# at-aaims/OmniFed

Measured on AMD Instinct MI355X. Metric: GB/s device-resident QSGD encode+decode, Llama-400M grads, 1/2/4/8 GPUs, higher is better.
Workload: dtype f32; 1 GPU; llama400m QSGD encode+decode, bit_width 4 (16 levels, int8 wire), philox draws, client weighting fused (alpha = batch_samples = rank + 1), one client per GPU; tensors=183, elements_per_client=401122304, bit_width=4, parallelism=clients1

## Files before the change

### omnifed_amd/csrc/omf_common.h

```cpp
#pragma once

#include <hip/hip_runtime.h>
#include <stdint.h>

#include <cstdlib>
#include <string>

namespace omf {

constexpr int kThreads = 256;
constexpr int kWaves = kThreads / 64;

constexpr unsigned kOrderEventFlags = hipEventDisableTiming | hipEventDisableSystemFence;

struct TopkStats {
  int64_t calls = 0, exact = 0;
};

struct TopkKnobs {
  TopkStats stats;
  bool init = false;
  int32_t groups = 1;
  int32_t dbg = 0;
  int32_t force_fallback = 0;
  int64_t sample_runs = 0;
  float sure_z = 1.5f, sure_c = 2.0f;
  bool scatter_small = true;
  bool planned_scatter = true;
};

inline const char* knob(const char* name) {
#ifdef OMF_EXPERIMENTS
  return std::getenv(name);
#else
  (void)name;
  return nullptr;
#endif
}

void set_error(const std::string& msg);
int fail(int code, const std::string& msg);
int hip_fail(hipError_t e, const char* what);

#define OMF_HIP(call)                                   \
  do {                                                  \
    hipError_t e_ = (call);                             \
    if (e_ != hipSuccess) return ::omf::hip_fail(e_, #call); \
  } while (0)

struct DeviceGuard {
  int prev = -1;
  bool ok = false;
  explicit DeviceGuard(int dev) {
    if (hipGetDevice(&prev) != hipSuccess) prev = -1;
    ok = hipSetDevice(dev) == hipSuccess;
  }
  ~DeviceGuard() {
    if (prev >= 0) (void)hipSetDevice(prev);
  }
};


__device__ __forceinline__ double wave_sum_f64(double v) {
#pragma unroll
  for (int o = 32; o > 0; o >>= 1) v += __shfl_xor(v, o, 64);
  return v;
}

__device__ __forceinline__ double block_sum_f64(double v, double* lds ) {
  v = wave_sum_f64(v);
  const int lane = threadIdx.x & 63, wave = threadIdx.x >> 6;
  if (lane == 0) lds[wave] = v;
  __syncthreads();
  double s = lds[0];
#pragma unroll
  for (int w = 1; w < kWaves; ++w) s += lds[w];
  __syncthreads();
  return s;
}

__device__ __forceinline__ uint64_t ld_agent(const uint64_t* p) {
  return __hip_atomic_load(const_cast<uint64_t*>(p), __ATOMIC_RELAXED, __HIP_MEMORY_SCOPE_AGENT);
}
__device__ __forceinline__ void st_agent(uint64_t* p, uint64_t v) {
  __hip_atomic_store(p, v, __ATOMIC_RELAXED, __HIP_MEMORY_SCOPE_AGENT);
}
__device__ __forceinline__ uint32_t add_agent(uint32_t* p, uint32_t v) {
  return __hip_atomic_fetch_add(p, v, __ATOMIC_RELAXED, __HIP_MEMORY_SCOPE_AGENT);
}
__device__ __forceinline__ void drain_vmem() { asm volatile("s_waitcnt vmcnt(0)" ::: "memory"); }

#ifndef OMF_PHILOX_ROUNDS
#define OMF_PHILOX_ROUNDS 10
#endif
__device__ __forceinline__ uint4 philox4x32_10(uint4 c, uint32_t k0, uint32_t k1) {
#pragma unroll
  for (int r = 0; r < OMF_PHILOX_ROUNDS; ++r) {
    if (r) {
      k0 += 0x9E3779B9u;
      k1 += 0xBB67AE85u;
    }
    const uint64_t p0 = (uint64_t)0xD2511F53u * c.x;
    const uint64_t p1 = (uint64_t)0xCD9E8D57u * c.z;
    c = make_uint4(__builtin_amdgcn_bitop3_b32((uint32_t)(p1 >> 32), c.y, k0, 0x96), (uint32_t)p1,
                   __builtin_amdgcn_bitop3_b32((uint32_t)(p0 >> 32), c.w, k1, 0x96), (uint32_t)p0);
  }
  return c;
}

__device__ __forceinline__ float u24(uint32_t w) { return (float)(w & 0xFFFFFFu) * 5.9604644775390625e-08f; }

__device__ __forceinline__ float4 u24x4(uint32_t w0, uint32_t w1, uint32_t w2) {
  return make_float4(u24(w0), u24(__builtin_amdgcn_alignbit(w1, w0, 24)), u24(__builtin_amdgcn_alignbit(w2, w1, 16)),
                     (float)(w2 >> 8) * 5.9604644775390625e-08f);
}

__device__ __forceinline__ float div_markstein(float x, float d, float r) {
  float q = __fmul_rn(x, r);
  float e = fmaf(-q, d, x);
  q = fmaf(e, r, q);
  e = fmaf(-q, d, x);
  return fmaf(e, r, q);
}

__device__ __forceinline__ bool div_needs_exact(float x) {
  const float a = fabsf(x);
  return a != 0.0f && !(a >= 0x1p-96f);
}

typedef float f32x4_t __attribute__((ext_vector_type(4)));
__device__ __forceinline__ void store_nt(float* p, float4 v) {
  f32x4_t t = {v.x, v.y, v.z, v.w};
  __builtin_nontemporal_store(t, reinterpret_cast<f32x4_t*>(p));
}
__device__ __forceinline__ void store_nt(uint32_t* p, uint32_t v) { __builtin_nontemporal_store(v, p); }
typedef int i32x4_t __attribute__((ext_vector_type(4)));
__device__ __forceinline__ void store_nt(int32_t* p, int4 v) {
  i32x4_t t = {v.x, v.y, v.z, v.w};
  __builtin_nontemporal_store(t, reinterpret_cast<i32x4_t*>(p));
}

}
```

### omnifed_amd/csrc/omf_qsgd.hip

```cpp
#include <algorithm>
#include <cstdlib>
#include <cstring>
#include <vector>

#include "../../include/omf_codec.h"
#include "../../include/omf_codec_experimental.h"
#include "omf_common.h"
#include "omf_qsgd_dev.h"
#include "omf_ring.h"

using namespace omf;

namespace {

constexpr int kV = 16;
constexpr int64_t kSub = (int64_t)kV * kThreads * 4;
constexpr uint64_t kWaitTicks = 2000000ull;

enum : int32_t { kNorm = 0, kQuant = 1, kResident = 2 };

struct Item {
  int64_t begin, end;
  int32_t tensor, kind, chunk, pad;
};
// ... 488 lines not shown
  for (int64_t rb = (int64_t)part * PER_ROUND; rb < R; rb += (int64_t)parts * PER_ROUND) {
    float4 v[PASSES];
    bool live[PASSES];
    auto run_pos = [&](int i) {
      const int64_t r0 = rb + (int64_t)i * RPP + (threadIdx.x / LPR);
      const int64_t r = r0 < R ? r0 : 0;
      const int64_t lo = r * base + min(r, rem), len = base + (r < rem ? 1 : 0);
      return ((lo + (int64_t)(spec_hash((uint32_t)r, (uint32_t)t) % (uint32_t)(len - (RUN - 1)))) & ~(int64_t)3) + 4 * j;
    };
#pragma unroll
    for (int i = 0; i < PASSES; ++i) {
      live[i] = rb + (int64_t)i * RPP + (threadIdx.x / LPR) < R;
      v[i] = *reinterpret_cast<const float4*>(x + run_pos(i));
    }
    if (AQ) {
#pragma unroll
      for (int i = 0; i < PASSES; ++i) v[i] = br_value(a, v[i], tb + run_pos(i), tb + n, t);
    }
#pragma unroll
    for (int i = 0; i < PASSES; ++i) {
      float sr = live[i] ? sq4(spec_prologue(v[i], alpha, a.divisor, a.e.fmt), 0.0f) : 0.0f;
#pragma unroll
      for (int o = LPR / 2; o > 0; o >>= 1) sr += __shfl_xor(sr, o, LPR);
      if (live[i] && j == 0) {
        s1 += (double)sr;
        s2 += (double)sr * (double)sr;
      }
    }
  }
}

__device__ SpecBracket bracket_from_sums(const SpecArgs& a, bool exact, int64_t n, int64_t R, int run, double S1,
                                         double S2);

template <bool WIDE, bool AQ>
__device__ __forceinline__ void spec_bracket_body(const SpecArgs& a, const SpecBrItem* __restrict__ items,
                                                  double* red, uint32_t& s_last) {
  const int parts = WIDE ? kBrParts : 1;
  const int part = (int)(blockIdx.x % (unsigned)parts);
  const SpecBrItem bi = items[blockIdx.x / (unsigned)parts];
  const int32_t t = bi.tensor;
  const int64_t tb = bi.begin, n = bi.n;
  const float* __restrict__ x = a.e.x + tb;
  const float alpha = a.e.alpha;
  double s1 = 0.0, s2 = 0.0;
  const bool exact = n <= kSpecExact;
  const int64_t R = WIDE ? (int64_t)bi.Rw : (int64_t)bi.R;
  if (exact) {
    constexpr int PER = (int)(kSpecExact / (4 * kBrThreads));
    float4 v[PER];
    const int64_t nq = n & ~(int64_t)3;
#pragma unroll
    for (int i = 0; i < PER; ++i) {
      const int64_t e = 4 * ((int64_t)i * kBrThreads + threadIdx.x);
      v[i] = nq ? *reinterpret_cast<const float4*>(x + (e < nq ? e : 0)) : make_float4(0.f, 0.f, 0.f, 0.f);
    }
#pragma unroll
    for (int i = 0; i < PER; ++i) {
      const int64_t e = 4 * ((int64_t)i * kBrThreads + threadIdx.x);
      if (e >= nq) {
        v[i] = make_float4(0.f, 0.f, 0.f, 0.f);
        if (e < n) {
          v[i].x = x[e];
          if (e + 1 < n) v[i].y = x[e + 1];
          if (e + 2 < n) v[i].z = x[e + 2];
        }
      }
    }
    if (AQ) {
#pragma unroll
      for (int i = 0; i < PER; ++i) {
        const int64_t e = 4 * ((int64_t)i * kBrThreads + threadIdx.x);
        if (e < n) v[i] = br_value(a, v[i], tb + e, tb + n, t);
      }
    }
    float acc = 0.0f;
#pragma unroll
    for (int i = 0; i < PER; ++i) acc = sq4(spec_prologue(v[i], alpha, a.divisor, a.e.fmt), acc);
    s1 = acc;
  } else {
    bracket_sample<WIDE ? kSpecRunWide : kSpecRun, AQ>(a, x, t, tb, n, R, part, parts, s1, s2);
  }
  if (exact && part != 0) return;
  double S1 = br_sum(s1, red);
  double S2 = br_sum(s2, red);
  if (!exact && parts > 1) {
    if (threadIdx.x == 0) {
      double* bp = a.br_part + 2 * ((int64_t)t * parts + part);
      st_agent(reinterpret_cast<uint64_t*>(bp), (uint64_t)__double_as_longlong(S1));
      st_agent(reinterpret_cast<uint64_t*>(bp + 1), (uint64_t)__double_as_longlong(S2));
      drain_vmem();
      const uint32_t last = add_agent(&a.br_cnt[t], 1u) == (uint32_t)(parts - 1) ? 1u : 0u;
      if (last) __hip_atomic_store(&a.br_cnt[t], 0u, __ATOMIC_RELAXED, __HIP_MEMORY_SCOPE_AGENT);
      s_last = last;
    }
    __syncthreads();
    if (!s_last || threadIdx.x != 0) return;
    S1 = S2 = 0.0;
    for (int g = 0; g < parts; ++g) {
      const uint64_t* bp = reinterpret_cast<const uint64_t*>(a.br_part + 2 * ((int64_t)t * parts + g));
      S1 += __longlong_as_double((long long)ld_agent(bp));
      S2 += __longlong_as_double((long long)ld_agent(bp + 1));
    }
  }
  if (threadIdx.x != 0) return;
  a.br[t] = bracket_from_sums(a, exact, n, R, WIDE ? kSpecRunWide : kSpecRun, S1, S2);
}

__device__ SpecBracket bracket_from_sums(const SpecArgs& a, bool exact, int64_t n, int64_t R, int run, double S1,
                                         double S2) {
  double ss, k;
  if (exact) {
    ss = S1;
    k = 0x1p-12;
  } else {
    const double Rd = (double)R, m = S1 / Rd;
    const double var = fmax(0.0, (S2 - Rd * m * m) / (Rd - 1.0));
    ss = S1 * ((double)n / ((double)run * Rd));
    k = (double)a.zsig * sqrt(var / Rd) / m + 0x1p-10;
  }
  const uint32_t fmt = a.e.fmt;
  const double kf = fmt == kFmtBF16 ? 0x1p-7 + 0x1p-14 : (fmt == kFmtF16 ? 0x1p-10 + 0x1p-20 : 0.0);
  const double mf = fmt == kFmtBF16 ? 0x1p-8 + 0x1p-16 : (fmt == kFmtF16 ? 0x1p-11 + 0x1p-22 : 0.0);
  k += kf;
  SpecBracket o{0.f, 0.f, 0.f, 0.f, 1u, {0u, 0u, 0u}};
  if (ss > 0.0 && ss < 1e300 && k < 0.5) {
    const float n_lo = nextafterf((float)sqrt(ss * (1.0 - k)), 0.0f);
    const float n_hi = nextafterf((float)sqrt(ss * (1.0 + k)), INFINITY);
    if (n_lo >= 0x1p-90f && n_hi < INFINITY) {
      const double L = (double)a.e.levels;
      o.n_lo = n_lo;
      o.n_hi = n_hi;
      o.c_lo = nextafterf((float)(L / (double)n_hi * (1.0 - 0x1p-20) * (1.0 - mf)), 0.0f);
      o.c_hi = nextafterf((float)(L / (double)n_lo * (1.0 + 0x1p-20) * (1.0 + mf)), INFINITY);
      o.mode = 0u;
    }
  }
  return o;
}

template <bool WIDE, bool AQ>
__global__ __launch_bounds__(kBrThreads) void qsgd_spec_bracket(SpecArgs a, const SpecBrItem* __restrict__ items) {
  __shared__ double red[kBrWaves];
  __shared__ uint32_t s_last;
  spec_bracket_body<WIDE, AQ>(a, items, red, s_last);
}
__global__ __launch_bounds__(kBrThreads) __attribute__((amdgpu_waves_per_eu(8))) void qsgd_spec_bracket_wide(
    SpecArgs a, const SpecBrItem* __restrict__ items) {
  __shared__ double red[kBrWaves];
  __shared__ uint32_t s_last;
  spec_bracket_body<true, false>(a, items, red, s_last);
}

__device__ __forceinline__ void spec_quad(float4 x, float4 u, float c_lo, float c_hi, int32_t (&q)[4], bool& und) {
  const float xs[4] = {x.x, x.y, x.z, x.w}, us[4] = {u.x, u.y, u.z, u.w};
#pragma unroll
  for (int c = 0; c < 4; ++c) {
    const float ax = fabsf(xs[c]);
    const float kl = ceilf(fmaf(ax, c_lo, -fmaxf(us[c], 0x1p-26f)));
    const float kh = ceilf(fmaf(ax, c_hi, -us[c]));
    und |= kl != kh;
    q[c] = (int32_t)copysignf(kh, xs[c]);
  }
}

__device__ __forceinline__ void spec_quad_fmt(float4 x, float4 u, float c_lo, float c_hi, float dl, int32_t (&q)[4],
                                              bool& und) {
  const float xs[4] = {x.x, x.y, x.z, x.w}, us[4] = {u.x, u.y, u.z, u.w};
#pragma unroll
  for (int c = 0; c < 4; ++c) {
    const float ax = fabsf(xs[c]);
    const float kl = ceilf(fmaf(ax, c_lo, -(fmaxf(us[c], 0x1p-26f) + dl)));
    const float kh = ceilf(fmaf(ax, c_hi, dl - us[c]));
    und |= kl != kh;
    q[c] = (int32_t)copysignf(kh, xs[c]);
  }
}

template <int WIDTH>
__device__ __forceinline__ void store_quad(const EncArgs& a, int64_t e, int64_t end, const int32_t (&qq)[4]) {
  if (WIDTH == 1) {
    int8_t* q8 = reinterpret_cast<int8_t*>(a.q);
    if (e + 4 <= end) {
      store_nt(reinterpret_cast<uint32_t*>(q8 + e), pack_i8x4(qq));
    } else {
      q8[e] = (int8_t)qq[0];
      if (e + 1 < end) q8[e + 1] = (int8_t)qq[1];
      if (e + 2 < end) q8[e + 2] = (int8_t)qq[2];
    }
  } else {
    int32_t* q32 = reinterpret_cast<int32_t*>(a.q);
    if (e + 4 <= end) {
      store_nt(q32 + e, make_int4(qq[0], qq[1], qq[2], qq[3]));
    } else {
      q32[e] = qq[0];
      if (e + 1 < end) q32[e + 1] = qq[1];
      if (e + 2 < end) q32[e + 2] = qq[2];
    }
  }
}

template <int WIDTH, bool FULL, bool DIV, uint32_t FMT, int AW = 0, int PW = kSpecPerWave, class GetBr>
__device__ __forceinline__ void spec_block(const SpecArgs& a, int64_t blk, int64_t b, int64_t end, int32_t t,
                                           int64_t tb, GetBr get_br, uint32_t* slot, uint64_t* part, float anorm,
                                           int tid) {
  const EncArgs& e = a.e;
  const int lane = tid & 63, wave = tid >> 6;
  float4 v[kSpecV];
  load_f4<kSpecV, FULL, true>(e.x, b, end, v, tid);
  int4 araw[AW ? kSpecV : 1];
  if (AW) {
#pragma unroll
    for (int k = 0; k < kSpecV; ++k)
      araw[k] = acc_load<AW ? AW : 1, FULL>(a.aq, b + 4 * ((int64_t)k * kThreads + tid), end);
  }
  float4 uu[4];
  philox_rows(e, b, tb, t, 0, uu, tid);
  const float alpha = e.alpha;
  float acc = 0.0f;
#pragma unroll
  for (int k = 0; k < kSpecV; ++k) {
    v[k].x = __fmul_rn(v[k].x, alpha); v[k].y = __fmul_rn(v[k].y, alpha);
    v[k].z = __fmul_rn(v[k].z, alpha); v[k].w = __fmul_rn(v[k].w, alpha);
    if (FMT != kFmtF32 && alpha != 1.0f) v[k] = round_fmt4(v[k], FMT);
    if (AW) {
      v[k] = acc_add4<AW ? AW : 1>(v[k], araw[k], anorm, a.alevels, a.ainv);
      if (a.aout) {
        const int64_t el = b + 4 * ((int64_t)k * kThreads + tid);
        if (FULL || el + 4 <= end) {
          store_nt(a.aout + el, v[k]);
        } else if (el < end) {
          a.aout[el] = v[k].x;
          if (el + 1 < end) a.aout[el + 1] = v[k].y;
          if (el + 2 < end) a.aout[el + 2] = v[k].z;
        }
      }
    }
    if (DIV) {
      const float d = a.divisor;
      v[k].x = __fdiv_rn(v[k].x, d); v[k].y = __fdiv_rn(v[k].y, d);
      v[k].z = __fdiv_rn(v[k].z, d); v[k].w = __fdiv_rn(v[k].w, d);
      const int64_t el = b + 4 * ((int64_t)k * kThreads + tid);
      if (FULL || el + 4 <= end) {
        store_nt(a.xout + el, v[k]);
      } else if (el < end) {
        a.xout[el] = v[k].x;
        if (el + 1 < end) a.xout[el + 1] = v[k].y;
        if (el + 2 < end) a.xout[el + 2] = v[k].z;
      }
    }
    acc = sq4(v[k], acc);
  }
  const SpecBracket br = get_br();
  uint32_t cnt = 0;
  {
    uint32_t* list = slot + PW * wave;
#pragma unroll
    for (int k = 0; k < kSpecV; ++k) {
      const int64_t el = b + 4 * ((int64_t)k * kThreads + tid);
      const bool live = FULL || el < end;
      int32_t qq[4];
      bool und = false;
      if (FMT == kFmtF32) spec_quad(v[k], uu[k], br.c_lo, br.c_hi, qq, und);
      else spec_quad_fmt(v[k], uu[k], br.c_lo, br.c_hi, FMT == kFmtF16 ? 0x1p-25f * e.levels : 0.0f, qq, und);
      if (live) store_quad<WIDTH>(e, el, FULL ? el + 4 : end, qq);
      const uint64_t m = __ballot(live && und);
      if (m) {
        const uint32_t pos = cnt + (uint32_t)__popcll(m & ((1ull << lane) - 1ull));
        if (live && und && pos < (uint32_t)PW) {
          list[pos] = (uint32_t)(el >> 2);
          float4* rec = a.recs + 2 * ((blk * kWaves + wave) * PW + pos);
          rec[0] = v[k];
          rec[1] = uu[k];
        }
        cnt += (uint32_t)__popcll(m);
      }
    }
  }
  const double s = wave_sum_f64((double)acc);
  if (lane == 0) {
    *part = (uint64_t)__double_as_longlong(s);
    a.heads[blk * kWaves + wave] = ((uint32_t)t << 8) | min(cnt, (uint32_t)PW);
    if (cnt > (uint32_t)PW)
      __hip_atomic_fetch_or(&a.flags[t], 1u, __ATOMIC_RELAXED, __HIP_MEMORY_SCOPE_AGENT);
  }
}

template <int WIDTH, bool DIV, uint32_t FMT = kFmtF32, int AW = 0, int PW = kSpecPerWave, int WPB = kWaves>
__global__ __launch_bounds__(64 * WPB) void qsgd_spec_quant(SpecArgs a, const SpecBracket* __restrict__ brs,
                                                            const int64_t* __restrict__ begins,
                                                            const float* __restrict__ anorms) {
  static_assert(kWaves % WPB == 0, "a block's waves split evenly");
  constexpr int kPer = kWaves / WPB;
  const int64_t blk = blockIdx.x / kPer;
  const int tid = (int)(blockIdx.x % kPer) * 64 * WPB + (int)threadIdx.x;
  const Item it = a.e.items[blk >> 2];
  const SpecBracket br = brs[it.tensor];
  const int64_t tb = begins[it.tensor];
  const float anorm = AW ? anorms[it.tensor] : 0.0f;
  const int64_t b = it.begin + (blk & 3) * kSpecBlk;
  const int wave = tid >> 6;
  uint32_t* slot = a.slots + blk * spec_slot_words(PW);
  uint64_t* part = a.partials + blk * kWaves + wave;
  if (b >= it.end) {
    if ((tid & 63) == 0) {
      *part = 0ull;
      a.heads[blk * kWaves + wave] = (uint32_t)it.tensor << 8;
    }
    return;
  }
  const int64_t end = min(b + kSpecBlk, it.end);
  auto get_br = [&]() { return br; };
  if (end - b == kSpecBlk)
    spec_block<WIDTH, true, DIV, FMT, AW, PW>(a, blk, b, end, it.tensor, tb, get_br, slot, part, anorm, tid);
  else
    spec_block<WIDTH, false, DIV, FMT, AW, PW>(a, blk, b, end, it.tensor, tb, get_br, slot, part, anorm, tid);
}

constexpr int kFbParts = 8;

__device__ __forceinline__ void spec_bracket_part(const SpecArgs& a, const SpecBrItem* __restrict__ items, int64_t wg) {
  __shared__ double red[kWaves];
  __shared__ uint32_t s_last;
  const int part = (int)(wg % kFbParts);
  const SpecBrItem bi = items[wg / kFbParts];
  const int32_t t = bi.tensor;
  const int64_t tb = bi.begin, n = bi.n, R = bi.R;
  const float* __restrict__ x = a.e.x + tb;
  const bool exact = n <= kSpecExact;
  if (exact && part != 0) return;
  double s1 = 0.0, s2 = 0.0;
  if (exact) {
    for (int64_t r0 = 0; r0 < n; r0 += 16 * kThreads) {
      float4 v[4];
#pragma unroll
      for (int i = 0; i < 4; ++i) {
        const int64_t e = r0 + 4 * ((int64_t)i * kThreads + threadIdx.x);
        v[i] = e + 4 <= n ? *reinterpret_cast<const float4*>(x + e) : make_float4(0.f, 0.f, 0.f, 0.f);
        if (e < n && e + 4 > n) {
          v[i].x = x[e];
          if (e + 1 < n) v[i].y = x[e + 1];
          if (e + 2 < n) v[i].z = x[e + 2];
        }
      }
      float acc = 0.0f;
#pragma unroll
      for (int i = 0; i < 4; ++i) acc = sq4(spec_prologue(v[i], a.e.alpha, a.divisor, a.e.fmt), acc);
      s1 += (double)acc;
    }
  } else {
    bracket_sample<kSpecRun, false, kThreads, 4>(a, x, t, tb, n, R, part, kFbParts, s1, s2);
  }
  double S1 = block_sum_f64(s1, red), S2 = block_sum_f64(s2, red);
  if (!exact) {
    if (threadIdx.x == 0) {
      double* bp = a.br_part + 2 * ((int64_t)t * kFbParts + part);
      st_agent(reinterpret_cast<uint64_t*>(bp), (uint64_t)__double_as_longlong(S1));
      st_agent(reinterpret_cast<uint64_t*>(bp + 1), (uint64_t)__double_as_longlong(S2));
      drain_vmem();
      const uint32_t last = add_agent(&a.br_cnt[t], 1u) == (uint32_t)(kFbParts - 1) ? 1u : 0u;
      if (last) __hip_atomic_store(&a.br_cnt[t], 0u, __ATOMIC_RELAXED, __HIP_MEMORY_SCOPE_AGENT);
      s_last = last;
    }
    __syncthreads();
    if (!s_last) return;
    S1 = S2 = 0.0;
    for (int g = 0; g < kFbParts; ++g) {
      const uint64_t* bp = reinterpret_cast<const uint64_t*>(a.br_part + 2 * ((int64_t)t * kFbParts + g));
      S1 += __longlong_as_double((long long)ld_agent(bp));
      S2 += __longlong_as_double((long long)ld_agent(bp + 1));
    }
  }
  if (threadIdx.x != 0) return;
  const SpecBracket o = bracket_from_sums(a, exact, n, R, kSpecRun, S1, S2);
  a.br[t] = o;
  const uint64_t ep = (uint64_t)a.epoch << 32;
  st_agent(&a.brgran[2 * t], ep | __float_as_uint(o.c_lo));
  st_agent(&a.brgran[2 * t + 1], ep | __float_as_uint(o.c_hi));
}

template <int WIDTH, bool DIV>
__global__ __launch_bounds__(kThreads) void qsgd_spec_quant_fb(SpecArgs a, const SpecBrItem* __restrict__ bitems,
                                                               int64_t nbrw, const int64_t* __restrict__ begins) {
  if ((int64_t)blockIdx.x < nbrw) {
    spec_bracket_part(a, bitems, blockIdx.x);
    return;
  }
  const int64_t blk = (int64_t)blockIdx.x - nbrw;
  const Item it = a.e.items[blk >> 2];
  const int32_t t = it.tensor;
  const int64_t tb = begins[t];
  const int64_t b = it.begin + (blk & 3) * kSpecBlk;
  const int wave = threadIdx.x >> 6;
  uint32_t* slot = a.slots + blk * kSpecSlot;
  uint64_t* part = a.partials + blk * kWaves + wave;
  if (b >= it.end) {
    if ((threadIdx.x & 63) == 0) {
      *part = 0ull;
      a.heads[blk * kWaves + wave] = (uint32_t)t << 8;
    }
    return;
  }
  auto get_br = [&]() {
    uint64_t g0 = ld_agent(&a.brgran[2 * t]), g1 = ld_agent(&a.brgran[2 * t + 1]);
    if ((uint32_t)(g0 >> 32) != a.epoch || (uint32_t)(g1 >> 32) != a.epoch) {
      const uint64_t t0 = wall_clock64(), min_polls = a.wait_ticks >> 10;
      uint64_t polls = 0;
      for (int k = 0;; k = min(k + 1, 6)) {
        if (k < 2) __builtin_amdgcn_s_sleep(2);
        else __builtin_amdgcn_s_sleep(8);
        g0 = ld_agent(&a.brgran[2 * t]);
        g1 = ld_agent(&a.brgran[2 * t + 1]);
        if ((uint32_t)(g0 >> 32) == a.epoch && (uint32_t)(g1 >> 32) == a.epoch) break;
        if (++polls > min_polls && wall_clock64() - t0 > a.wait_ticks) {
          __hip_atomic_fetch_or(&a.flags[t], 2u, __ATOMIC_RELAXED, __HIP_MEMORY_SCOPE_AGENT);
          g0 = g1 = 0;
          break;
        }
      }
    }
    SpecBracket o{__uint_as_float((uint32_t)g0), __uint_as_float((uint32_t)g1), 0.f, 0.f, 0u, {0u, 0u, 0u}};
// ... 1353 lines not shown
}

struct AccIn {
  const void* q;
  int32_t width, levels;
  const float* norm;
  float* acc_out;
};

static int encode_launch(omf_plan* p, const float* x, float alpha, int32_t s, const float* u, uint64_t seed,
                         uint64_t offset, const float* norm_in, void* q, float* norm_out, bool norm_only, void* stream,
                         float divisor, float* xout, uint32_t fmt, const AccIn* acc_in);

static int encode_impl(omf_plan* p, const float* x, float alpha, int32_t s, const float* u, uint64_t seed,
                       uint64_t offset, const float* norm_in, void* q, float* norm_out, bool norm_only, void* stream,
                       float divisor = 0.0f, float* xout = nullptr, int32_t fmt = 0, const AccIn* acc_in = nullptr) {
  if (!p) return fail(OMF_EINVAL, "plan is NULL");
  if (fmt < 0 || fmt > 2) return fail(OMF_EINVAL, "value_format must be 0 (fp32), 1 (bf16) or 2 (fp16)");
  DeviceGuard g(p->device);
  if (!g.ok) return fail(OMF_EHIP, "hipSetDevice failed");
  if (int r = plan_enter(p, (hipStream_t)stream)) return r;
  if (int r = encode_launch(p, x, alpha, s, u, seed, offset, norm_in, q, norm_out, norm_only, stream, divisor, xout,
                            (uint32_t)fmt, acc_in))
    return r;
  return plan_leave(p, (hipStream_t)stream);
}

static bool spec_serves(const omf_plan* p, int32_t s, const float* u, float divisor, uint32_t fmt, bool wide_ok);

static int encode_launch(omf_plan* p, const float* x, float alpha, int32_t s, const float* u, uint64_t seed,
                         uint64_t offset, const float* norm_in, void* q, float* norm_out, bool norm_only, void* stream,
                         float divisor, float* xout, uint32_t fmt, const AccIn* acc_in) {
  if (!p) return fail(OMF_EINVAL, "plan is NULL");
  if (int r = check_bits(s)) return r;
  const int width = (1 << s) <= 127 ? 1 : 4;
  if (!x || !norm_out || (!norm_only && !q)) return fail(OMF_EINVAL, "x, q and norm_out must be non-NULL");
  if (!aligned(x, 16) || (u && !aligned(u, 16)) || (q && !aligned(q, width == 1 ? 4 : 16)))
    return fail(OMF_EINVAL, "misaligned buffer (fp32/int32 need 16 B, int8 needs 4 B alignment)");
  DeviceGuard g(p->device);
  if (!g.ok) return fail(OMF_EHIP, "hipSetDevice failed");
  hipStream_t st = (hipStream_t)stream;
  EncArgs a;
  a.x = x; a.u = u; a.norm_in = norm_in; a.q = q; a.norm_out = norm_out;
  a.partials = p->d_partials;
  a.ticket = reinterpret_cast<uint32_t*>(p->d_sync);
  a.err = reinterpret_cast<uint32_t*>(p->d_sync + 4);
  a.counters = reinterpret_cast<uint32_t*>(p->d_sync + p->off_counters);
  a.gran = reinterpret_cast<uint64_t*>(p->d_sync + p->off_gran);
  a.alpha = alpha;
  a.fmt = fmt;
  a.levels = (float)(1u << s);
  a.seed_lo = (uint32_t)seed; a.seed_hi = (uint32_t)(seed >> 32); a.offset = (uint32_t)offset;
  a.wait_ticks = p->wait_ticks;
  const dim3 blk(kThreads);
  if (norm_in && !norm_only) {
    a.items = p->d_flat;
    a.tinfo = p->d_tinfo[0];
    const dim3 grid4((unsigned)(p->n_flat * 4));
    p->last_encoder = 5;
    if (width == 1) {
      if (u) hipLaunchKernelGGL((qsgd_quant_sub<1, true, 4, false>), grid4, blk, 0, st, a);
      else hipLaunchKernelGGL((qsgd_quant_sub<1, false, 4, false>), grid4, blk, 0, st, a);
    } else {
      if (u) hipLaunchKernelGGL((qsgd_quant_sub<4, true, 4, false>), grid4, blk, 0, st, a);
      else hipLaunchKernelGGL((qsgd_quant_sub<4, false, 4, false>), grid4, blk, 0, st, a);
    }
    OMF_HIP(hipGetLastError());
    return OMF_OK;
  }
  if (p->strategy == 4 && !norm_only && !u && divisor == 0.0f && p->grid_wgs > 0 &&
      p->n_spec_blocks <= (int64_t)p->grid_wgs * 4 * kGridNB) {
    GridArgs ga;
    a.items = p->d_flat;
    ga.e = a;
    ga.partials = p->d_spec_part;
    ga.bar = p->d_grid_bar;
    ga.target = (unsigned long long)(p->grid_launches + 1) * (unsigned long long)p->grid_wgs;
    ga.nblocks = p->n_spec_blocks;
    ga.dbg = p->spec_skip;
    const dim3 gg((unsigned)p->grid_wgs), gblk(1024);
    if (width == 1)
      hipLaunchKernelGGL(qsgd_encode_grid<1>, gg, gblk, 0, st, ga, (const Item*)p->d_flat, (const int64_t*)p->d_begins,
                         (const uint32_t*)p->d_grid_pbeg, (const uint32_t*)p->d_grid_pcnt);
    else
      hipLaunchKernelGGL(qsgd_encode_grid<4>, gg, gblk, 0, st, ga, (const Item*)p->d_flat, (const int64_t*)p->d_begins,
                         (const uint32_t*)p->d_grid_pbeg, (const uint32_t*)p->d_grid_pcnt);
    OMF_HIP(hipGetLastError());
    ++p->grid_launches;
    p->last_encoder = 4;
    return OMF_OK;
  }
  if (!norm_only && spec_serves(p, s, u, divisor, fmt, acc_in == nullptr)) {
    SpecArgs sa;
    a.items = p->d_flat;
    a.tinfo = p->d_tinfo[1];
    sa.e = a;
    p->last_encoder = 3;
    sa.begins = p->d_begins;
    sa.sizes = p->d_sizes;
    sa.br_items = p->d_spec_br_items;
    sa.fold_items = p->d_spec_fold_items;
    sa.seg_part = p->d_spec_seg_part;
    sa.fold_cnt = p->d_spec_cnt;
    if (++p->spec_epoch >= 0x80000000u) p->spec_epoch = 1;
    sa.epoch = p->spec_epoch;
    sa.wide = s > kSpecMaxBits ? 1u : 0u;
    sa.ngran = p->d_spec_ngran;
    sa.dbg = p->spec_skip;
    sa.zsig = s > kSpecMaxBits ? p->spec_zsig_wide : p->spec_zsig;
    sa.divisor = divisor;
    sa.xout = xout;
    sa.wait_ticks = p->wait_ticks;
    sa.br = p->d_spec_br;
    sa.partials = p->d_spec_part;
    const bool wide = s > kSpecMaxBits;
    if (wide && !p->d_spec_slots_w) {
      OMF_HIP(hipMalloc(&p->d_spec_slots_w, 4 * (size_t)spec_slot_words(kSpecPerWaveWide) * (size_t)p->n_spec_blocks));
      OMF_HIP(hipMalloc(&p->d_spec_recs_w, 32 * (size_t)kWaves * kSpecPerWaveWide * (size_t)p->n_spec_blocks));
      OMF_HIP(hipMalloc(&p->d_spec_br_part, 16 * (size_t)kBrParts * (size_t)p->nt));
      OMF_HIP(hipMalloc(&p->d_spec_br_cnt, 4 * (size_t)p->nt));
      OMF_HIP(hipMemsetAsync(p->d_spec_br_cnt, 0, 4 * (size_t)p->nt, st));
    }
    const bool fb = p->spec_fb && !wide && !acc_in && fmt == 0 && width == 1 && !(p->spec_skip & 1u);
    const bool wfb = p->spec_fb && wide && !acc_in && fmt == 0 && !(p->spec_skip & 1u);
    if ((fb || wfb) && !p->d_spec_fb_part) {
      OMF_HIP(hipMalloc(&p->d_spec_fb_part, 16 * (size_t)std::max(kFbParts, kWfbParts) * (size_t)p->nt));
      OMF_HIP(hipMalloc(&p->d_spec_fb_cnt, 4 * (size_t)p->nt));
      OMF_HIP(hipMalloc(&p->d_spec_brgran, 16 * (size_t)p->nt));
      OMF_HIP(hipMemsetAsync(p->d_spec_fb_cnt, 0, 4 * (size_t)p->nt, st));
      OMF_HIP(hipMemsetAsync(p->d_spec_brgran, 0, 16 * (size_t)p->nt, st));
    }
    sa.br_part = fb || wfb ? p->d_spec_fb_part : p->d_spec_br_part;
    sa.br_cnt = fb || wfb ? p->d_spec_fb_cnt : p->d_spec_br_cnt;
    sa.brgran = p->d_spec_brgran;
    p->spec_last_pw = wide ? kSpecPerWaveWide : kSpecPerWave;
    sa.slots = wide ? p->d_spec_slots_w : p->d_spec_slots;
    sa.heads = p->d_spec_heads;
    sa.recs = wide ? p->d_spec_recs_w : p->d_spec_recs;
    sa.flags = p->d_spec_flags;
    sa.status = p->d_spec_status;
    sa.nblocks = p->n_spec_blocks;
    sa.aq = acc_in ? acc_in->q : nullptr;
    sa.anorm = acc_in ? acc_in->norm : nullptr;
    sa.aout = acc_in ? acc_in->acc_out : nullptr;
    sa.awidth = acc_in ? acc_in->width : 0;
    sa.alevels = acc_in ? (float)acc_in->levels : 0.0f;
    sa.ainv = acc_in && (acc_in->levels & (acc_in->levels - 1)) == 0 ? 1.0f / (float)acc_in->levels : 0.0f;
    const dim3 gbr((unsigned)(p->n_spec_br * (s > kSpecMaxBits ? kBrParts : 1))), gb((unsigned)p->n_spec_blocks);
    const bool div = divisor != 0.0f;
    static const size_t plds_w = [] { const char* v = omf::knob("OMF_SPEC_LDS_W"); return v ? (size_t)atoi(v) : (size_t)10240; }();
    if (fb) {
      const int64_t nbrw = (int64_t)kFbParts * p->n_spec_br;
      const dim3 gfb((unsigned)(nbrw + p->n_spec_blocks));
      if (div) hipLaunchKernelGGL((qsgd_spec_quant_fb<1, true>), gfb, blk, 0, st, sa, sa.br_items, nbrw, sa.begins);
      else hipLaunchKernelGGL((qsgd_spec_quant_fb<1, false>), gfb, blk, 0, st, sa, sa.br_items, nbrw, sa.begins);
    } else if (wfb) {
      const int64_t nbrw = (int64_t)kWfbParts * p->n_spec_br;
      const dim3 gw((unsigned)(nbrw + p->n_spec_blocks * kWaves)), bw(64);
      if (width == 1 && !div) hipLaunchKernelGGL((qsgd_spec_quant_wfb<1, false>), gw, bw, plds_w, st, sa, sa.br_items, nbrw, sa.begins);
      else if (width == 1) hipLaunchKernelGGL((qsgd_spec_quant_wfb<1, true>), gw, bw, plds_w, st, sa, sa.br_items, nbrw, sa.begins);
      else if (!div) hipLaunchKernelGGL((qsgd_spec_quant_wfb<4, false>), gw, bw, plds_w, st, sa, sa.br_items, nbrw, sa.begins);
      else hipLaunchKernelGGL((qsgd_spec_quant_wfb<4, true>), gw, bw, plds_w, st, sa, sa.br_items, nbrw, sa.begins);
    } else if (!(p->spec_skip & 1u)) {
      if (wide) hipLaunchKernelGGL(qsgd_spec_bracket_wide, gbr, dim3(kBrThreads), 0, st, sa, sa.br_items);
      else if (sa.aq) hipLaunchKernelGGL((qsgd_spec_bracket<false, true>), gbr, dim3(kBrThreads), 0, st, sa, sa.br_items);
      else hipLaunchKernelGGL((qsgd_spec_bracket<false, false>), gbr, dim3(kBrThreads), 0, st, sa, sa.br_items);
    }
    const float* an = sa.anorm;
    const int aw = acc_in ? (acc_in->width == 32 ? 4 : 1) : 0;
    constexpr int PWW = kSpecPerWaveWide;
    if (fb || wfb) {
    } else if (wide) {
      static const bool wpb4 = [] { const char* v = omf::knob("OMF_SPEC_WPB"); return v && atoi(v) == 4; }();
      const dim3 g1((unsigned)(p->n_spec_blocks * kWaves)), b1(64);
      if (wpb4) {
        if (width == 1 && !div) hipLaunchKernelGGL((qsgd_spec_quant<1, false, kFmtF32, 0, PWW>), gb, blk, 0, st, sa, sa.br, sa.begins, an);
        else if (width == 1) hipLaunchKernelGGL((qsgd_spec_quant<1, true, kFmtF32, 0, PWW>), gb, blk, 0, st, sa, sa.br, sa.begins, an);
        else if (!div) hipLaunchKernelGGL((qsgd_spec_quant<4, false, kFmtF32, 0, PWW>), gb, blk, 0, st, sa, sa.br, sa.begins, an);
        else hipLaunchKernelGGL((qsgd_spec_quant<4, true, kFmtF32, 0, PWW>), gb, blk, 0, st, sa, sa.br, sa.begins, an);
      } else {
        if (width == 1 && !div) hipLaunchKernelGGL((qsgd_spec_quant<1, false, kFmtF32, 0, PWW, 1>), g1, b1, plds_w, st, sa, sa.br, sa.begins, an);
        else if (width == 1) hipLaunchKernelGGL((qsgd_spec_quant<1, true, kFmtF32, 0, PWW, 1>), g1, b1, plds_w, st, sa, sa.br, sa.begins, an);
        else if (!div) hipLaunchKernelGGL((qsgd_spec_quant<4, false, kFmtF32, 0, PWW, 1>), g1, b1, plds_w, st, sa, sa.br, sa.begins, an);
        else hipLaunchKernelGGL((qsgd_spec_quant<4, true, kFmtF32, 0, PWW, 1>), g1, b1, plds_w, st, sa, sa.br, sa.begins, an);
      }
    } else if (fmt == kFmtBF16) hipLaunchKernelGGL((qsgd_spec_quant<1, false, kFmtBF16>), gb, blk, 0, st, sa, sa.br, sa.begins, an);
    else if (fmt == kFmtF16) hipLaunchKernelGGL((qsgd_spec_quant<1, false, kFmtF16>), gb, blk, 0, st, sa, sa.br, sa.begins, an);
    else if (width == 1 && !div) hipLaunchKernelGGL((qsgd_spec_quant<1, false>), gb, blk, 0, st, sa, sa.br, sa.begins, an);
    else if (width == 1 && aw == 1) hipLaunchKernelGGL((qsgd_spec_quant<1, true, kFmtF32, 1>), gb, blk, 0, st, sa, sa.br, sa.begins, an);
    else if (width == 1 && aw == 4) hipLaunchKernelGGL((qsgd_spec_quant<1, true, kFmtF32, 4>), gb, blk, 0, st, sa, sa.br, sa.begins, an);
    else if (width == 1) hipLaunchKernelGGL((qsgd_spec_quant<1, true>), gb, blk, 0, st, sa, sa.br, sa.begins, an);
    else if (!div) hipLaunchKernelGGL((qsgd_spec_quant<4, false>), gb, blk, 0, st, sa, sa.br, sa.begins, an);
    else hipLaunchKernelGGL((qsgd_spec_quant<4, true>), gb, blk, 0, st, sa, sa.br, sa.begins, an);
    if (p->spec_skip & 2u) {
      OMF_HIP(hipGetLastError());
      return OMF_OK;
    }
    const int32_t nfold = (int32_t)p->n_spec_fold;
    if (wide) {
#ifndef OMF_FIX_FT
#define OMF_FIX_FT 4
#endif
      constexpr int FT = OMF_FIX_FT, BPW = kThreads / (kWaves * FT);
      const dim3 gw((unsigned)(nfold + (p->n_spec_blocks + BPW - 1) / BPW));
      if (width == 1)
        hipLaunchKernelGGL((qsgd_spec_finish<1, PWW, FT>), gw, blk, 0, st, sa, (const SpecFoldItem*)sa.fold_items, nfold,
                           (const Item*)a.items, (const int64_t*)sa.begins, (const uint32_t*)sa.slots,
                           (const float4*)sa.recs, (const uint32_t*)sa.heads);
      else
        hipLaunchKernelGGL((qsgd_spec_finish<4, PWW, FT>), gw, blk, 0, st, sa, (const SpecFoldItem*)sa.fold_items, nfold,
                           (const Item*)a.items, (const int64_t*)sa.begins, (const uint32_t*)sa.slots,
                           (const float4*)sa.recs, (const uint32_t*)sa.heads);
      OMF_HIP(hipGetLastError());
      return OMF_OK;
    }
    const dim3 gfin((unsigned)(nfold + (p->n_spec_blocks + kThreads / kWaves - 1) / (kThreads / kWaves)));
    if (width == 1)
      hipLaunchKernelGGL(qsgd_spec_finish<1>, gfin, blk, 0, st, sa, (const SpecFoldItem*)sa.fold_items, nfold,
                         (const Item*)a.items, (const int64_t*)sa.begins, (const uint32_t*)sa.slots,
                         (const float4*)sa.recs, (const uint32_t*)sa.heads);
    else
      hipLaunchKernelGGL(qsgd_spec_finish<4>, gfin, blk, 0, st, sa, (const SpecFoldItem*)sa.fold_items, nfold,
                         (const Item*)a.items, (const int64_t*)sa.begins, (const uint32_t*)sa.slots,
                         (const float4*)sa.recs, (const uint32_t*)sa.heads);
    OMF_HIP(hipGetLastError());
    return OMF_OK;
  }
  const bool wide_ring = p->strategy == 3 && width == 4 && !u && fmt == 0;
  if ((p->strategy == 2 || p->strategy == 4 || divisor != 0.0f || wide_ring) && !norm_only) {
    omf::ring::Args r;
    r.x = x; r.u = u; r.q = q; r.norm_out = norm_out;
    r.items = p->d_ring; r.tinfo = p->d_ring_t; r.gran = p->d_ring_gran;
    r.err = reinterpret_cast<uint32_t*>(p->d_sync + 4);
    r.n_items = p->n_ring;
    r.alpha = alpha;
    r.fmt = fmt;
    r.round_in = (fmt != 0 && alpha != 1.0f) ? 1u : 0u;
    r.divisor = divisor;
    r.divide = divisor != 0.0f ? 1u : 0u;
    r.xout = xout;
    r.levels = (float)(1u << s);
    r.seed_lo = (uint32_t)seed; r.seed_hi = (uint32_t)(seed >> 32); r.offset = (uint32_t)offset;
    if (++p->ring_epoch == 0) ++p->ring_epoch;
    r.epoch = p->ring_epoch;
    r.wait_ticks = p->wait_ticks;
    r.lds_wait_ticks = p->lds_wait_ticks;
    r.dbg = p->ring_dbg;
    r.prof = p->d_ring_prof;
    const int grid = (int)std::min<int64_t>(p->ring_grid, std::max<int64_t>(p->n_ring, 1));
    p->last_encoder = 2;
    if (omf::ring::launch(p->ring_cfg, width, u != nullptr, r, grid, st) != 0)
      return fail(OMF_EHIP, "ring encoder launch failed");
    OMF_HIP(hipGetLastError());
    return OMF_OK;
  }
  const int strat = p->strategy >= 2 ? 1 : p->strategy;
  if (++p->epoch == 0) ++p->epoch;
  a.epoch = p->epoch;
  a.n_items = (uint32_t)p->n_enc[strat];
  a.items = p->d_enc[strat];
  a.tinfo = p->d_tinfo[strat];
  const dim3 grid((unsigned)p->n_enc[strat]);
  if (!norm_only) p->last_encoder = strat;
#define OMF_ENC(EV)                                                                              \
  do {                                                                                           \
    if (norm_only) {                                                                             \
      hipLaunchKernelGGL((qsgd_encode_ordered<1, false, true, EV>), grid, blk, 0, st, a);        \
    } else if (width == 1) {                                                                     \
      if (u) hipLaunchKernelGGL((qsgd_encode_ordered<1, true, false, EV>), grid, blk, 0, st, a); \
      else hipLaunchKernelGGL((qsgd_encode_ordered<1, false, false, EV>), grid, blk, 0, st, a);  \
    } else {                                                                                     \
      if (u) hipLaunchKernelGGL((qsgd_encode_ordered<4, true, false, EV>), grid, blk, 0, st, a); \
      else hipLaunchKernelGGL((qsgd_encode_ordered<4, false, false, EV>), grid, blk, 0, st, a);  \
    }                                                                                            \
  } while (0)
  if (p->ev == 8) OMF_ENC(8);
  else OMF_ENC(16);
#undef OMF_ENC
  OMF_HIP(hipGetLastError());
  return OMF_OK;
}

static bool spec_serves(const omf_plan* p, int32_t s, const float* u, float divisor, uint32_t fmt, bool wide_ok) {
  if (p->strategy != 3 || u || s < kSpecMinBits) return false;
  if (s <= kSpecMaxBits) return fmt == 0 || divisor == 0.0f;
  return wide_ok && p->spec_wide && s <= kSpecMaxBitsWide && fmt == 0;
}

int omf_qsgd_encode(omf_plan* plan, const float* x, float alpha, int32_t bit_width, const float* u, uint64_t seed,
                    uint64_t offset, const float* norm_in, void* q_out, float* norm_out, void* stream) {
  return encode_impl(plan, x, alpha, bit_width, u, seed, offset, norm_in, q_out, norm_out, false, stream);
}

int omf_qsgd_encode_ex(omf_plan* plan, const float* x, float alpha, int32_t bit_width, int32_t value_format,
                       const float* u, uint64_t seed, uint64_t offset, const float* norm_in, void* q_out,
                       float* norm_out, void* stream) {
  return encode_impl(plan, x, alpha, bit_width, u, seed, offset, norm_in, q_out, norm_out, false, stream, 0.0f,
                     nullptr, value_format);
}

int omf_qsgd_norms_ex(omf_plan* plan, const float* x, float alpha, int32_t value_format, float* norm_out,
                      void* stream) {
  return encode_impl(plan, x, alpha, 0, nullptr, 0, 0, nullptr, nullptr, norm_out, true, stream, 0.0f, nullptr,
                     value_format);
}

int omf_ps_apply_encode(omf_plan* p, const float* acc, float divisor, float* avg_out, int32_t bit_width,
                        const float* u, uint64_t seed, uint64_t offset, void* q_out, float* norm_out, void* stream) {
// ... 132 lines not shown
```

### omnifed_amd/csrc/omf_qsgd_dev.h

```cpp
#pragma once

#include "omf_common.h"

namespace omf {

typedef float f32x2_t __attribute__((ext_vector_type(2)));

enum : uint32_t { kFmtF32 = 0, kFmtBF16 = 1, kFmtF16 = 2 };

__device__ __forceinline__ float round_bf16(float f) {
  if (f != f) return f;
  const uint32_t u = __float_as_uint(f);
  return __uint_as_float((u + 0x7FFFu + ((u >> 16) & 1u)) & 0xFFFF0000u);
}
__device__ __forceinline__ float round_f16(float f) { return (float)(_Float16)f; }
__device__ __forceinline__ float round_fmt(float f, uint32_t fmt) {
  return fmt == kFmtBF16 ? round_bf16(f) : (fmt == kFmtF16 ? round_f16(f) : f);
}
__device__ __forceinline__ float4 round_fmt4(float4 v, uint32_t fmt) {
  return make_float4(round_fmt(v.x, fmt), round_fmt(v.y, fmt), round_fmt(v.z, fmt), round_fmt(v.w, fmt));
}
__device__ __forceinline__ float finish_norm(double sumsq, uint32_t fmt) { return round_fmt(sqrtf((float)sumsq), fmt); }

__device__ __forceinline__ f32x2_t fma2(f32x2_t a, f32x2_t b, f32x2_t c) { return __builtin_elementwise_fma(a, b, c); }

__device__ __forceinline__ f32x2_t div2_markstein(f32x2_t x, f32x2_t d, f32x2_t r) {
  f32x2_t q = x * r;
  f32x2_t e = fma2(-q, d, x);
  q = fma2(e, r, q);
  e = fma2(-q, d, x);
  return fma2(e, r, q);
}

__device__ __forceinline__ bool div_tiny(float x) { return __builtin_amdgcn_frexp_expf(x) < -95; }

struct Divisor {
  float d, r;
  bool fast;
  uint32_t fmt;
  __device__ __forceinline__ explicit Divisor(float norm, uint32_t fmt_ = kFmtF32) : d(norm), r(1.0f / norm), fmt(fmt_) {
    const float a = fabsf(norm);
    fast = a >= 0x1p-100f && a <= 0x1p100f;
  }
  __device__ __forceinline__ float4 div4(float4 x) const {
    const float4 q = div4_f32(x);
    return fmt ? round_fmt4(q, fmt) : q;
  }
  __device__ __forceinline__ float4 div4_f32(float4 x) const {
    if (!fast) return make_float4(x.x / d, x.y / d, x.z / d, x.w / d);
    const f32x2_t D = {d, d}, R = {r, r};
    const f32x2_t lo = div2_markstein((f32x2_t){x.x, x.y}, D, R);
    const f32x2_t hi = div2_markstein((f32x2_t){x.z, x.w}, D, R);
    float4 q = make_float4(lo.x, lo.y, hi.x, hi.y);
    const float mn = fminf(fminf(fabsf(x.x), fabsf(x.y)), fminf(fabsf(x.z), fabsf(x.w)));
    if (__any(mn < 0x1p-96f)) {
      if (div_tiny(x.x)) q.x = x.x / d;
      if (div_tiny(x.y)) q.y = x.y / d;
      if (div_tiny(x.z)) q.z = x.z / d;
      if (div_tiny(x.w)) q.w = x.w / d;
    }
    return q;
  }
};

__device__ __forceinline__ int32_t qsgd_level_fast(float vn, float L, float u) {
  const float a = fabsf(__fmul_rn(vn, L));
  const float fl = floorf(a);
  const float p = __fsub_rn(a, fl);
  float m = (u < p) ? __fadd_rn(fl, 1.0f) : fl;
  m = __builtin_elementwise_minimum(m, L);
  return (int32_t)copysignf(m, vn);
}

__device__ __forceinline__ int32_t qsgd_level(float vn, float L, float u) {
  const float a = fabsf(__fmul_rn(vn, L));
  if (!(a < 9.2233720e18f)) return 0;
  return qsgd_level_fast(vn, L, u);
}

template <bool CHECK_BIG = true>
__device__ __forceinline__ void qsgd_quad(float4 x, float4 u, const Divisor& dv, float L, bool zero,
                                          int32_t (&q)[4]) {
  if (zero) {
    q[0] = q[1] = q[2] = q[3] = 0;
    return;
  }
  const float4 vn = dv.div4(x);
  q[0] = qsgd_level_fast(vn.x, L, u.x);
  q[1] = qsgd_level_fast(vn.y, L, u.y);
  q[2] = qsgd_level_fast(vn.z, L, u.z);
  q[3] = qsgd_level_fast(vn.w, L, u.w);
  if (dv.fmt == kFmtF16) {
    if (!(fabsf(__fmul_rn(vn.x, L)) < 65520.0f)) q[0] = 0;
    if (!(fabsf(__fmul_rn(vn.y, L)) < 65520.0f)) q[1] = 0;
    if (!(fabsf(__fmul_rn(vn.z, L)) < 65520.0f)) q[2] = 0;
    if (!(fabsf(__fmul_rn(vn.w, L)) < 65520.0f)) q[3] = 0;
  }
  if (!CHECK_BIG) return;
  const float big = fmaxf(fmaxf(fabsf(vn.x), fabsf(vn.y)), fmaxf(fabsf(vn.z), fabsf(vn.w)));
  if (__any(!(__fmul_rn(big, L) < 9.2233720e18f) && big == big)) {
    if (!(fabsf(__fmul_rn(vn.x, L)) < 9.2233720e18f)) q[0] = 0;
    if (!(fabsf(__fmul_rn(vn.y, L)) < 9.2233720e18f)) q[1] = 0;
    if (!(fabsf(__fmul_rn(vn.z, L)) < 9.2233720e18f)) q[2] = 0;
    if (!(fabsf(__fmul_rn(vn.w, L)) < 9.2233720e18f)) q[3] = 0;
  }
}

__device__ __forceinline__ uint32_t pack_i8x4(const int32_t (&q)[4]) {
  return (uint32_t)(uint8_t)q[0] | ((uint32_t)(uint8_t)q[1] << 8) | ((uint32_t)(uint8_t)q[2] << 16) |
         ((uint32_t)(uint8_t)q[3] << 24);
}

}
```

Before: 6322 GB/s.

## Micro-optimize QSGD encode with permlane/DPP reductions, v_perm packing and mask ballots

Replaces the shuffle-based f64 wave reduction with permlane32/16 swaps plus DPP moves. It uses v_perm for the uniform-draw bit extraction and int8 packing, and replaces the bool ballot in spec_quad with a direct fcmp lane mask and mbcnt prefix count. It also makes the wave index scalar with readfirstlane and launches the non-div fallback quant kernel with 24 KB of dynamic LDS, which is likely meant to cap occupancy. These instruction-level tweaks target ALU and cross-lane overhead in a memory-bound kernel, and the new DPP/perm control codes carry correctness risk.

```diff
diff --git a/omnifed_amd/csrc/omf_common.h b/omnifed_amd/csrc/omf_common.h
--- a/omnifed_amd/csrc/omf_common.h
+++ b/omnifed_amd/csrc/omf_common.h
@@ -61,9 +61,37 @@
 };
 
 
+template <int CTRL>
+__device__ __forceinline__ uint32_t dpp_mov(uint32_t x) {
+  return (uint32_t)__builtin_amdgcn_update_dpp(0, (int)x, CTRL, 0xF, 0xF, true);
+}
+template <int CTRL>
+__device__ __forceinline__ double dpp_mov_f64(double v) {
+  const uint64_t b = (uint64_t)__double_as_longlong(v);
+  return __longlong_as_double((long long)(((uint64_t)dpp_mov<CTRL>((uint32_t)(b >> 32)) << 32) | dpp_mov<CTRL>((uint32_t)b)));
+}
+
 __device__ __forceinline__ double wave_sum_f64(double v) {
-#pragma unroll
-  for (int o = 32; o > 0; o >>= 1) v += __shfl_xor(v, o, 64);
+  {
+    const uint64_t b = (uint64_t)__double_as_longlong(v);
+    const uint32_t lo = (uint32_t)b, hi = (uint32_t)(b >> 32);
+    const auto l = __builtin_amdgcn_permlane32_swap(lo, lo, false, false);
+    const auto h = __builtin_amdgcn_permlane32_swap(hi, hi, false, false);
+    v = __longlong_as_double((long long)(((uint64_t)h[0] << 32) | l[0])) +
+        __longlong_as_double((long long)(((uint64_t)h[1] << 32) | l[1]));
+  }
+  {
+    const uint64_t b = (uint64_t)__double_as_longlong(v);
+    const uint32_t lo = (uint32_t)b, hi = (uint32_t)(b >> 32);
+    const auto l = __builtin_amdgcn_permlane16_swap(lo, lo, false, false);
+    const auto h = __builtin_amdgcn_permlane16_swap(hi, hi, false, false);
+    v = __longlong_as_double((long long)(((uint64_t)h[0] << 32) | l[0])) +
+        __longlong_as_double((long long)(((uint64_t)h[1] << 32) | l[1]));
+  }
+  v += dpp_mov_f64<0x128>(v);
+  v += dpp_mov_f64<0x1B>(dpp_mov_f64<0x141>(v));
+  v += dpp_mov_f64<0x4E>(v);
+  v += dpp_mov_f64<0xB1>(v);
   return v;
 }
 
@@ -111,8 +139,10 @@
 __device__ __forceinline__ float u24(uint32_t w) { return (float)(w & 0xFFFFFFu) * 5.9604644775390625e-08f; }
 
 __device__ __forceinline__ float4 u24x4(uint32_t w0, uint32_t w1, uint32_t w2) {
-  return make_float4(u24(w0), u24(__builtin_amdgcn_alignbit(w1, w0, 24)), u24(__builtin_amdgcn_alignbit(w2, w1, 16)),
-                     (float)(w2 >> 8) * 5.9604644775390625e-08f);
+  constexpr float k = 5.9604644775390625e-08f;
+  return make_float4(u24(w0), (float)__builtin_amdgcn_perm(w1, w0, 0x0c050403u) * k,
+                     (float)__builtin_amdgcn_perm(w2, w1, 0x0c040302u) * k,
+                     (float)(w2 >> 8) * k);
 }
 
 __device__ __forceinline__ float div_markstein(float x, float d, float r) {
diff --git a/omnifed_amd/csrc/omf_qsgd.hip b/omnifed_amd/csrc/omf_qsgd.hip
--- a/omnifed_amd/csrc/omf_qsgd.hip
+++ b/omnifed_amd/csrc/omf_qsgd.hip
@@ -664,27 +664,30 @@
   spec_bracket_body<true, false>(a, items, red, s_last);
 }
 
-__device__ __forceinline__ void spec_quad(float4 x, float4 u, float c_lo, float c_hi, int32_t (&q)[4], bool& und) {
+__device__ __forceinline__ float raise_u(float u) {
+  return __uint_as_float(max(__float_as_uint(u), 0x32800000u));
+}
+__device__ __forceinline__ void spec_quad(float4 x, float4 u, float c_lo, float c_hi, int32_t (&q)[4], uint64_t& und) {
   const float xs[4] = {x.x, x.y, x.z, x.w}, us[4] = {u.x, u.y, u.z, u.w};
 #pragma unroll
   for (int c = 0; c < 4; ++c) {
     const float ax = fabsf(xs[c]);
-    const float kl = ceilf(fmaf(ax, c_lo, -fmaxf(us[c], 0x1p-26f)));
+    const float kl = ceilf(fmaf(ax, c_lo, -raise_u(us[c])));
     const float kh = ceilf(fmaf(ax, c_hi, -us[c]));
-    und |= kl != kh;
+    und |= __builtin_amdgcn_fcmpf(kl, kh, 14 );
     q[c] = (int32_t)copysignf(kh, xs[c]);
   }
 }
 
 __device__ __forceinline__ void spec_quad_fmt(float4 x, float4 u, float c_lo, float c_hi, float dl, int32_t (&q)[4],
-                                              bool& und) {
+                                              uint64_t& und) {
   const float xs[4] = {x.x, x.y, x.z, x.w}, us[4] = {u.x, u.y, u.z, u.w};
 #pragma unroll
   for (int c = 0; c < 4; ++c) {
     const float ax = fabsf(xs[c]);
-    const float kl = ceilf(fmaf(ax, c_lo, -(fmaxf(us[c], 0x1p-26f) + dl)));
+    const float kl = ceilf(fmaf(ax, c_lo, -(raise_u(us[c]) + dl)));
     const float kh = ceilf(fmaf(ax, c_hi, dl - us[c]));
-    und |= kl != kh;
+    und |= __builtin_amdgcn_fcmpf(kl, kh, 14 );
     q[c] = (int32_t)copysignf(kh, xs[c]);
   }
 }
@@ -717,7 +720,8 @@
                                            int64_t tb, GetBr get_br, uint32_t* slot, uint64_t* part, float anorm,
                                            int tid) {
   const EncArgs& e = a.e;
-  const int lane = tid & 63, wave = tid >> 6;
+  const int lane = tid & 63;
+  const int wave = __builtin_amdgcn_readfirstlane(tid >> 6);
   float4 v[kSpecV];
   load_f4<kSpecV, FULL, true>(e.x, b, end, v, tid);
   int4 araw[AW ? kSpecV : 1];
@@ -772,13 +776,15 @@
       const int64_t el = b + 4 * ((int64_t)k * kThreads + tid);
       const bool live = FULL || el < end;
       int32_t qq[4];
-      bool und = false;
-      if (FMT == kFmtF32) spec_quad(v[k], uu[k], br.c_lo, br.c_hi, qq, und);
-      else spec_quad_fmt(v[k], uu[k], br.c_lo, br.c_hi, FMT == kFmtF16 ? 0x1p-25f * e.levels : 0.0f, qq, und);
+      uint64_t m = 0;
+      if (FMT == kFmtF32) spec_quad(v[k], uu[k], br.c_lo, br.c_hi, qq, m);
+      else spec_quad_fmt(v[k], uu[k], br.c_lo, br.c_hi, FMT == kFmtF16 ? 0x1p-25f * e.levels : 0.0f, qq, m);
       if (live) store_quad<WIDTH>(e, el, FULL ? el + 4 : end, qq);
-      const uint64_t m = __ballot(live && und);
+      if (!FULL) m &= __builtin_amdgcn_ballot_w64(live);
       if (m) {
-        const uint32_t pos = cnt + (uint32_t)__popcll(m & ((1ull << lane) - 1ull));
+        const bool und = (m >> lane) & 1ull;
+        const uint32_t pos =
+            cnt + __builtin_amdgcn_mbcnt_hi((uint32_t)(m >> 32), __builtin_amdgcn_mbcnt_lo((uint32_t)m, 0u));
         if (live && und && pos < (uint32_t)PW) {
           list[pos] = (uint32_t)(el >> 2);
           float4* rec = a.recs + 2 * ((blk * kWaves + wave) * PW + pos);
@@ -2438,8 +2444,9 @@
     if (fb) {
       const int64_t nbrw = (int64_t)kFbParts * p->n_spec_br;
       const dim3 gfb((unsigned)(nbrw + p->n_spec_blocks));
+      static const size_t plds_n = [] { const char* v = omf::knob("OMF_SPEC_LDS"); return v ? (size_t)atoi(v) : (size_t)24576; }();
       if (div) hipLaunchKernelGGL((qsgd_spec_quant_fb<1, true>), gfb, blk, 0, st, sa, sa.br_items, nbrw, sa.begins);
-      else hipLaunchKernelGGL((qsgd_spec_quant_fb<1, false>), gfb, blk, 0, st, sa, sa.br_items, nbrw, sa.begins);
+      else hipLaunchKernelGGL((qsgd_spec_quant_fb<1, false>), gfb, blk, plds_n, st, sa, sa.br_items, nbrw, sa.begins);
     } else if (wfb) {
       const int64_t nbrw = (int64_t)kWfbParts * p->n_spec_br;
       const dim3 gw((unsigned)(nbrw + p->n_spec_blocks * kWaves)), bw(64);
diff --git a/omnifed_amd/csrc/omf_qsgd_dev.h b/omnifed_amd/csrc/omf_qsgd_dev.h
--- a/omnifed_amd/csrc/omf_qsgd_dev.h
+++ b/omnifed_amd/csrc/omf_qsgd_dev.h
@@ -107,8 +107,8 @@
 }
 
 __device__ __forceinline__ uint32_t pack_i8x4(const int32_t (&q)[4]) {
-  return (uint32_t)(uint8_t)q[0] | ((uint32_t)(uint8_t)q[1] << 8) | ((uint32_t)(uint8_t)q[2] << 16) |
-         ((uint32_t)(uint8_t)q[3] << 24);
+  return __builtin_amdgcn_perm((uint32_t)q[1], (uint32_t)q[0], 0x0c0c0400u) |
+         __builtin_amdgcn_perm((uint32_t)q[3], (uint32_t)q[2], 0x04000c0cu);
 }
 
 }
```

New measurement: 6409 GB/s, median of 6. 1.4% higher.
